# balkce/beamform

Measured on AMD Instinct MI355X. Metric: stft_frames_per_sec, higher is better.
Workload: dtype f64; 1 GPU; das 8-mic 1024-pt (hop 512), 65536-frame batch per GPU, 1 stream(s), planar input resident in HBM; frames_per_gpu=65536, frames_fed_per_gpu=65536, mics=8, fft=1024, hop=512, streams=1, layout=planar, gather=n/a, parallelism=independent batches x1, input=uniform noise in [-0.5, 0.5), settle_launches_before_warmup=408, forward_transforms_per_frame_pair=6

## Files before the change

### beamform_amd/csrc/das_f64_plan.hpp

```cpp
#pragma once

#include <cstdlib>
#include <cstring>

#include "../../include/bfcore.h"

#if defined(__HIPCC__)
#define BF_PLAN_HD __host__ __device__ inline
#else
#define BF_PLAN_HD inline
#endif

namespace bf {

constexpr int kChunkEnd = 0xFFFFF;
constexpr int kMaxChunkPairs = 1000;
constexpr int kSchedMaxChunks = 16384;
constexpr size_t kSchedCounterBytes = 256, kSchedRowBytes = 16;
constexpr size_t das_f64_sched_ws_bytes() { return kSchedCounterBytes + kSchedMaxChunks * kSchedRowBytes; }
constexpr int kDasF64Hop = 512, kDasF64Waves = 8, kDasF64RingSlots = 40;

struct DasSchedPlan {
    int n_levels;
    int cnt[8], size[8];
    int n_chunks;
    int grid;
};

BF_PLAN_HD void das_f64_chunk(const DasSchedPlan &p, long n_frames, int n_streams, int k, int *stream, long *t0, long *n) {
    int lvl = 0, kk = k;
    long pair0 = 0;
    while (lvl < p.n_levels - 1 && kk >= p.cnt[lvl] * n_streams) {
        kk -= p.cnt[lvl] * n_streams;
        pair0 += (long)p.cnt[lvl] * p.size[lvl];
        ++lvl;
    }
    const int s = kk / p.cnt[lvl], j = kk - s * p.cnt[lvl];
    *stream = s;
    *t0 = 2 * (pair0 + (long)j * p.size[lvl]);
    long len = 2L * p.size[lvl];
    if (*t0 + len > n_frames) len = n_frames - *t0;
    *n = len;
}

inline DasSchedPlan das_f64_plan(long n_frames, int n_streams, int n_cus, const char *env) {
    DasSchedPlan p{};
    const long pairs = (n_frames + 1) / 2;
    long nb = (long)n_cus / n_streams;
    if (nb < 1) nb = 1;
    int sizes[8], n_sizes = 0;
    const long share = (pairs + nb - 1) / nb;
    if (env && strchr(env, ',')) {
        const char *c = env;
        while (*c && n_sizes < 8) {
            sizes[n_sizes++] = atoi(c);
            c = strchr(c, ',');
            if (!c) break;
            ++c;
        }
    } else if (!(env && atoi(env) == 0) && share >= 48) {
        long front = (share * 13 / 16) & ~7L;
        long rest = share - front;
        while (front > kMaxChunkPairs && n_sizes < 3) {
            sizes[n_sizes++] = kMaxChunkPairs;
            front -= kMaxChunkPairs;
        }
        if (front > kMaxChunkPairs) { rest += front - kMaxChunkPairs; front = kMaxChunkPairs; }
        sizes[n_sizes++] = (int)front;
        while (n_sizes < 6 && rest >= 24) {
            long sz = (rest / 2) & ~7L;
            if (sz > kMaxChunkPairs) sz = kMaxChunkPairs;
            sizes[n_sizes++] = (int)sz;
            rest -= sz;
        }
        if (rest >= 12) { sizes[n_sizes++] = 4; rest -= 4; }
// ... 77 lines not shown
```

### beamform_amd/csrc/das_f64_w64.hip

```cpp
#include <hip/hip_runtime.h>

#include <type_traits>

#include "launch_trace.hpp"
#include "pipeline_kernels.hpp"
#include "w64_f64_dev.hpp"

namespace bf {

namespace {

constexpr int kBlock = 512;
constexpr int kWaves = kBlock / 64;
constexpr int kHop = 512;
constexpr int kTwD = 2 * (1024 + 4 * kTw2RowW64Rot);
constexpr int oTw = 0;
constexpr int oPlane = kTwD;
constexpr int oGain = oPlane + kWaves * kPlaneD;
constexpr int oCross = oGain + 4 * 2048;
constexpr int oFlag = oCross + 512;
constexpr int kWinRow = 18;
constexpr int oWin = oFlag + 8;
constexpr int kLdsD = oWin + 64 * kWinRow;

typedef volatile __attribute__((address_space(3))) int *lds_flag_t;

template <int LAYOUT>
__global__ __launch_bounds__(kBlock) void das_f64_w64_kernel(DasF64Args a, int frames_per_chunk, int chunks_per_stream) {
    __shared__ __attribute__((aligned(16))) double lds[kLdsD];
    const cx<double> *s_tw1 = reinterpret_cast<const cx<double> *>(lds + oTw);
    const cx<double> *s_tw2 = s_tw1 + 1024;
    const cx<double> *s_gain = reinterpret_cast<const cx<double> *>(lds + oGain);
    float *s_cross = reinterpret_cast<float *>(lds + oCross);
    lds_flag_t s_ready = (lds_flag_t)(lds + oFlag);
    lds_flag_t s_cons = s_ready + kWaves;

    const int tid = threadIdx.x, lane = tid & 63;
    const int w = __builtin_amdgcn_readfirstlane(tid >> 6);
    const int M = a.n_mics, NP = (M + 1) >> 1;
    double *plane = lds + oPlane + w * kPlaneD;
    double *wcol = plane + w64_col_rot(lane);
    double *row16 = plane + (lane & 15) * kRS + 16 * (lane >> 4);

    const int stream = blockIdx.x / chunks_per_stream;
    const long c_in_s = blockIdx.x - (long)stream * chunks_per_stream;
    const double *wrow = lds + oWin + lane * kWinRow;

    const long T0 = c_in_s * frames_per_chunk;
    long T1 = T0 + frames_per_chunk;
    if (T1 > a.n_frames) T1 = a.n_frames;
    const float *xs = a.x + (long)stream * a.stream_stride_x;
    const float *hs = a.hist + (long)stream * M * kHop;
    float *ys = a.y + (long)stream * a.n_frames * kHop;

    float na[16], nb[16];
    auto request = [&](long tt, int p) {
        const int ma = 2 * p, mb = (2 * p + 1 < M) ? 2 * p + 1 : ma;
        if (LAYOUT == 0) {
// ... 6 lines not shown
                na[j] = a1[(unsigned)(64 * j + lane)];
                nb[j] = b1[(unsigned)(64 * j + lane)];
                na[j + 8] = a2[(unsigned)(64 * j + lane)];
                nb[j + 8] = b2[(unsigned)(64 * j + lane)];
            }
        } else {
            const float *s1 = tt >= 1 ? xs + (tt - 1) * (long)kHop * M : hs;
            const float *s2 = xs + tt * (long)kHop * M;
            if ((M & 1) == 0) {
#pragma unroll
                for (int j = 0; j < 8; ++j) {
                    const float2 v1 = *reinterpret_cast<const float2 *>(s1 + (unsigned)((64 * j + lane) * M + ma));
                    const float2 v2 = *reinterpret_cast<const float2 *>(s2 + (unsigned)((64 * j + lane) * M + ma));
                    na[j] = v1.x;
                    nb[j] = v1.y;
                    na[j + 8] = v2.x;
                    nb[j + 8] = v2.y;
                }
            } else {
#pragma unroll
                for (int j = 0; j < 8; ++j) {
                    na[j] = s1[(unsigned)((64 * j + lane) * M + ma)];
                    nb[j] = s1[(unsigned)((64 * j + lane) * M + mb)];
                    na[j + 8] = s2[(unsigned)((64 * j + lane) * M + ma)];
                    nb[j + 8] = s2[(unsigned)((64 * j + lane) * M + mb)];
                }
            }
        }
    };

    const int n_iter = (int)((T1 - T0 + kWaves - 1) / kWaves);
    if (T0 + w < T1) request(T0 + w, 0);
    {
        const f64x2 *tw2 = a.tw, *g2 = a.gains;
        f64x2 *ltw = reinterpret_cast<f64x2 *>(lds + oTw), *lg = reinterpret_cast<f64x2 *>(lds + oGain);
#pragma unroll 4
        for (int i = tid; i < kTwD / 2; i += kBlock) ltw[i] = tw2[i];
#pragma unroll 8
        for (int i = tid; i < NP * 1024; i += kBlock) lg[i] = g2[i];
#pragma unroll 2
        for (int i = tid; i < 1024; i += kBlock) lds[oWin + (i & 63) * kWinRow + (i >> 6)] = a.win[i];
        if (tid < 2 * kWaves) s_ready[tid] = -2;
    }
    __syncthreads();
    for (int it = 0; it < n_iter; ++it) {
        const long t = T0 + (long)it * kWaves + w;
        if (t >= T1) break;

        double Sr[16], Si[16];
        for (int p = 0; p < NP; ++p) {
            double re[16], im[16];
            const bool b_ok = 2 * p + 1 < M;
#pragma unroll
            for (int j = 0; j < 8; ++j) {
                const double w0 = wrow[j], w1 = wrow[j + 8];
                const double t = (double)na[j] * w0, u = (double)na[j + 8];
                re[j] = fma(u, w1, t);
                re[j + 8] = fma(-u, w1, t);
            }
            if (b_ok) {
#pragma unroll
                for (int j = 0; j < 8; ++j) {
                    const double w0 = wrow[j], w1 = wrow[j + 8];
                    const double t = (double)nb[j] * w0, u = (double)nb[j + 8];
                    im[j] = fma(u, w1, t);
                    im[j + 8] = fma(-u, w1, t);
                }
            } else {
#pragma unroll
                for (int j = 0; j < 16; ++j) im[j] = 0.0;
            }
            {
                long tn = t;
                int pn = p + 1;
// ... 119 lines not shown
                float *yn = ys + T1 * kHop;
#pragma unroll
                for (int j = 0; j < 8; ++j) atomicAdd(yn + (unsigned)(64 * j + lane), o[j + 8]);
            } else {
                float *to = a.tail_out + (long)stream * kHop;
#pragma unroll
                for (int j = 0; j < 8; ++j) to[(unsigned)(64 * j + lane)] = o[j + 8];
            }
        }
    }
}


#ifdef BF_PARK_PLAIN
#define BF_PARK_LD(p) (*(const volatile float *)(p))
#else
#define BF_PARK_LD(p) __builtin_nontemporal_load(p)
#endif
constexpr int kGRow = 65;
constexpr int kGMic = 8 * kGRow;
constexpr int kSlots = 64;
constexpr int kTwP = 2 * (960 + 4 * kTw2RowW64Rot);
constexpr int pTw = 0;
constexpr int pPlane = kTwP;
constexpr int pGain = pPlane + kWaves * kPlaneD;
constexpr int pFlag = pGain + 7 * kGMic * 2;
constexpr int kRingR = 32;
constexpr int kRingSlots = kRingR + kWaves;
constexpr int pRing = pFlag + (kSlots + 4) / 2;
constexpr int pWin = pRing + kRingR / 2;
constexpr int kLdsP = pWin + 64 * kWinRow;
static_assert(kLdsP * 8 <= 160 * 1024, "LDS");
static_assert((pGain & 1) == 0 && (pWin & 1) == 0, "16-byte alignment");


typedef volatile __attribute__((address_space(3))) int *lds_int_t;
typedef volatile __attribute__((address_space(3))) unsigned long long *lds_u64_t;
__device__ __forceinline__ int lds_fetch_add(lds_int_t p, int v, int lane) {
    int old = 0;
    if (lane == 0) old = __hip_atomic_fetch_add((__attribute__((address_space(3))) int *)p, v, __ATOMIC_RELAXED, __HIP_MEMORY_SCOPE_WORKGROUP);
    return __builtin_amdgcn_readfirstlane(old);
}
__device__ __forceinline__ unsigned long long lds_fetch_add64(lds_u64_t p, int lane) {
    unsigned long long old = 0;
    if (lane == 0) old = __hip_atomic_fetch_add((__attribute__((address_space(3))) unsigned long long *)p, 1ull, __ATOMIC_RELAXED, __HIP_MEMORY_SCOPE_WORKGROUP);
    const unsigned lo = (unsigned)__builtin_amdgcn_readfirstlane((int)(unsigned)old), hi = (unsigned)__builtin_amdgcn_readfirstlane((int)(unsigned)(old >> 32));
    return ((unsigned long long)hi << 32) | lo;
}
struct DasSched {
    const int4 *chunks;
    unsigned *counter;
    int n_chunks;
};
__device__ __forceinline__ unsigned long long pack_work(unsigned vbase, int chunk, int pairs, int next) {
    return ((unsigned long long)(vbase & 0xFFFFFFu) << 40) | ((unsigned long long)(unsigned)chunk << 20) | ((unsigned long long)(unsigned)pairs << 10) | (unsigned)next;
}
struct PairWork {
    int4 d;
    int pos;
    int len;
    unsigned u;
    bool have;
};
__device__ __forceinline__ int4 load_chunk(const int4 *chunks, int k) {
    const int4 d = chunks[k];
    return int4{__builtin_amdgcn_readfirstlane(d.x), __builtin_amdgcn_readfirstlane(d.y), __builtin_amdgcn_readfirstlane(d.z), k};
}
__device__ __forceinline__ PairWork draw_pair(lds_u64_t work, const DasSched &sc, int lane, const int4 held) {
    PairWork r;
    r.have = false;
    r.d = int4{0, 0, 0, 0};
    r.pos = r.len = 0;
    r.u = 0;
    for (;;) {
        const unsigned long long old = lds_fetch_add64(work, lane);
        const int pos = (int)(old & 1023u), len = (int)((old >> 10) & 1023u), k = (int)((old >> 20) & 0xFFFFFu);
        const unsigned vb = (unsigned)(old >> 40);
        if (k == kChunkEnd) return r;
        if (pos < len) {
            if (k == held.w) r.d = held;
            else r.d = load_chunk(sc.chunks, k);
            r.pos = pos; r.len = len; r.u = vb + (unsigned)pos; r.have = true;
            return r;
        }
        if (pos == len) {
// ... 208 lines not shown
            r.h = ring_slot(jp);
        }
        __builtin_amdgcn_fence(__ATOMIC_ACQUIRE, "workgroup");
        return r;
    };
    auto release_pair = [&](const PairWork &pw, bool has_t) {
        const unsigned u2 = 2u * pw.u;
        (void)lds_fetch_add(s_ring + (u2 & (kRingR - 1)), 2, lane);
        (void)lds_fetch_add(s_ring + ((u2 + 1) & (kRingR - 1)), has_t ? 1 : 2, lane);
        if (pw.pos > 0) (void)lds_fetch_add(s_ring + ((u2 - 1) & (kRingR - 1)), 1, lane);
    };
    auto request_ring_mic = [&](const RingHops &r, int m) { request(r.h + m * kHop, r.a + m * kHop, r.b + m * kHop); };
    auto request_ring_extra = [&](bool on, const RingHops &r) {
        if (!on) {
#pragma unroll
            for (int j = 0; j < 8; ++j) e0[j] = e1[j] = e2[j] = 0.f;
            return;
        }
#pragma unroll
        for (int j = 0; j < 8; ++j) {
            e0[j] = r.h[XM * kHop + (unsigned)(64 * j + lane)];
            e1[j] = r.a[XM * kHop + (unsigned)(64 * j + lane)];
            e2[j] = r.b[XM * kHop + (unsigned)(64 * j + lane)];
        }
    };
    RingHops curR{nullptr, nullptr, nullptr};
    (void)curR;

    BF_STAMP(0);
#ifdef BF_W64_STAMPS
    if (lane == 0 && blockIdx.x < 256) g_stamps[(blockIdx.x * 8 + w) * 64 + 59] = __builtin_amdgcn_s_memtime();
#endif
    PairWork cur;
    cur.d = load_chunk(sc.chunks, (int)blockIdx.x);
    cur.len = (cur.d.z + 1) >> 1;
    const int n_static = cur.len < kWaves ? cur.len : kWaves;
    cur.pos = w;
    cur.u = (unsigned)w;
    cur.have = w < n_static;
    if (LAYOUT == 0 && cur.have) {
        request_pair_mic(cur.d.x, cur.d.y + 2L * w, a.slot_mic[0]);
        request_extra(XM >= 0, cur.d.x, cur.d.y + 2L * w);
    } else {
        request_extra(false, 0, 0);
    }
    {
        const f64x2 *tw2 = a.tw + 64;
        f64x2 *ltw = reinterpret_cast<f64x2 *>(lds + pTw), *lg = reinterpret_cast<f64x2 *>(lds + pGain);
#pragma unroll 4
        for (int i = tid; i < kTwP / 2; i += kBlock) ltw[i] = tw2[i];
        for (int k = 0; k < NT; ++k) {
            const f64x2 *g2 = a.gains_mic + a.slot_mic[k] * kGMic;
#pragma unroll 2
            for (int i = tid; i < kGMic; i += kBlock) lg[k * kGMic + i] = g2[i];
        }
#pragma unroll 2
        for (int i = tid; i < 1024; i += kBlock) lds[pWin + (i & 63) * kWinRow + (i >> 6)] = a.win[i];
        if (tid < kSlots) s_state[tid] = 0;
        if (tid < kRingR) s_ring[tid] = 0;
        if (tid == 0) *s_work = pack_work(0u, (int)blockIdx.x, cur.len, n_static);
    }
    __syncthreads();
    BF_STAMP(1);
    BF_STATS_DECL;
    int it = 0;
    if (!cur.have) {
        cur = draw_pair(s_work, sc, lane, cur.d);
        if (LAYOUT == 0 && cur.have) {
            request_pair_mic(cur.d.x, cur.d.y + 2L * cur.pos, a.slot_mic[0]);
            request_extra(XM >= 0, cur.d.x, cur.d.y + 2L * cur.pos);
        }
    }
    while (cur.have) {
        if constexpr (LAYOUT == 1) {
            curR = prepare_pair(cur);
            request_ring_mic(curR, a.slot_mic[0]);
            request_ring_extra(XM >= 0, curR);
        }
        const int stream = cur.d.x;
        const long T0 = cur.d.y, T1 = T0 + cur.d.z;
        const long tA = T0 + 2L * cur.pos;
        const bool pair = tA + 1 < T1;
        const long tL = pair ? tA + 1 : tA;
        const unsigned u = cur.u;
        const bool has_t = cur.pos + 1 < cur.len, has_h = cur.pos > 0;
        float *ys = a.y + (long)stream * a.n_frames * kHop;
        PairWork nxt;
        nxt.have = false;
        const float *hp0 = a.x + (long)stream * a.stream_stride_x + tA * kHop;
        const float *hist0 = a.hist + (long)stream * M * kHop;
// ... 295 lines not shown
    const float4 *src = reinterpret_cast<const float4 *>(x + s * in_stream_stride + tile * 256 * M);
    const int R = M + 1;
    for (int i = tid; i < 64 * M; i += 256) {
        const float4 v = src[i];
        const int e = 4 * i;
        s_t[(e / M) * R + e % M] = v.x;
        s_t[((e + 1) / M) * R + (e + 1) % M] = v.y;
        s_t[((e + 2) / M) * R + (e + 2) % M] = v.z;
        s_t[((e + 3) / M) * R + (e + 3) % M] = v.w;
    }
    __syncthreads();
    float *dst = out + s * out_stream_stride + tile * 256;
    for (int j = tid; j < 64 * M; j += 256) {
        const int m = j >> 6, q = j & 63;
        const float4 v{s_t[(4 * q) * R + m], s_t[(4 * q + 1) * R + m], s_t[(4 * q + 2) * R + m], s_t[(4 * q + 3) * R + m]};
        reinterpret_cast<float4 *>(dst + (long)m * out_mic_stride)[q] = v;
    }
}

}

static_assert(kWaves == kDasF64Waves && kRingSlots == kDasF64RingSlots && kHop == kDasF64Hop, "das_f64_plan.hpp describes other kernels");
static_assert(sizeof(int4) == kSchedRowBytes, "a row of the chunk table is one int4");

static hipError_t launch_interleaved_to_planar(const float *x, float *out, long n, int n_mics, int n_streams, hipStream_t s) {
    const long tiles = n / 256;
    BF_LAUNCH(interleaved_to_planar_kernel, dim3((unsigned)(tiles * n_streams)), dim3(256), 0, s, x, out, tiles, n_mics, (long)n_mics * n, n, (long)n_mics * n);
    return hipGetLastError();
}

hipError_t enqueue_das_f64(DasF64Args a, const DasF64Launch &d, float *scratch, hipStream_t s, hipEvent_t kev0, hipEvent_t kev1, bool *kev_recorded) {
    hipError_t e = hipSuccess;
    int4 *const chunks = reinterpret_cast<int4 *>(reinterpret_cast<char *>(a.sched_ws) + kSchedCounterBytes);
    const DasSched sc{chunks, reinterpret_cast<unsigned *>(a.sched_ws), d.plan.n_chunks};
    if (d.path == DasF64Path::kMicPair) {
        for (int st = 0; st < a.n_streams && d.runs_per_stream > 1; ++st) {
            e = hipMemset2DAsync(a.y + ((long)st * a.n_frames + d.run_frames) * kHop, (size_t)d.run_frames * kHop * sizeof(float), 0, kHop * sizeof(float), (size_t)d.runs_per_stream - 1, s);
            if (e != hipSuccess) return e;
        }
    } else {
        if (d.path == DasF64Path::kRing) {
            a.ring = scratch; a.ring_bytes = d.scratch_bytes; a.hist_out = nullptr;
        } else if (d.path == DasF64Path::kTranspose) {
            const long n = a.n_frames * kHop;
            float *const hist = scratch + (size_t)a.n_streams * a.n_mics * n;
            if ((e = launch_interleaved_to_planar(a.x, scratch, n, a.n_mics, a.n_streams, s)) != hipSuccess) return e;
            if ((e = launch_interleaved_to_planar(a.hist, hist, kHop, a.n_mics, a.n_streams, s)) != hipSuccess) return e;
            a.x = scratch; a.hist = hist; a.hist_out = nullptr; a.mic_stride = n; a.layout = BF_PLANAR;
        }
        BF_LAUNCH(das_f64_sched_kernel, dim3((unsigned)((sc.n_chunks + kSchedPerBlock - 1) / kSchedPerBlock)), dim3(32 * kSchedPerBlock), 0, s, d.plan, chunks, sc.counter, a.y, a.n_frames, a.n_streams);
        if ((e = hipGetLastError()) != hipSuccess) return e;
    }
    if (kev0 && (e = hipEventRecord(kev0, s)) != hipSuccess) return e;
    if (d.path == DasF64Path::kMicPair)
        BF_LAUNCH(das_f64_w64_kernel<1>, dim3((unsigned)(d.runs_per_stream * a.n_streams)), dim3(kBlock), 0, s, a, (int)d.run_frames, (int)d.runs_per_stream);
    else if (d.path == DasF64Path::kRing)
        BF_LAUNCH(das_f64_ring_kernel, dim3((unsigned)d.plan.grid), dim3(kBlock), 0, s, a, sc);
    else
        BF_LAUNCH(das_f64_pair_kernel, dim3((unsigned)d.plan.grid), dim3(kBlock), 0, s, a, sc);
    if ((e = hipGetLastError()) != hipSuccess) return e;
    if (kev1 && (e = hipEventRecord(kev1, s)) == hipSuccess) *kev_recorded = true;
    return e;
}

}

#ifdef BF_W64_STATS
// ... 10 lines not shown
```

### beamform_amd/csrc/pipeline.hip

```cpp
#include "pipeline.hpp"

#include <hip/hip_runtime.h>

#include <cmath>
#include <vector>

#include "device_mem.hpp"
#include "fft1024.hpp"
#include "pipeline_kernels.hpp"
#include "switches.hpp"

namespace bf {

namespace {

class BinPipelineImpl : public Engine {
    static constexpr int kMaxCols = BF_MAX_INTERF + 1;
   public:
    BinPipelineImpl(const bf_config &c, int n_cus) : cfg_(c), n_cus_(n_cus) {
        M_ = c.n_mics;
        H_ = c.hop;
        N_ = 2 * c.hop;
        NQ_ = problems_per_frame(N_);
        YS_ = yh_stride(N_);
        ks_ = kernel_set(N_);
        MF_ = single_ch_ ? 1 : M_;
        NP_ = (MF_ + 1) / 2;
        S_ = c.n_streams;
        D_ = c.n_dirs > 1 ? c.n_dirs : 1;
        if (time_node_) D_ = M_;
        So_ = S_ * D_;
        R_ = (c.algo == BF_GSS && c.gss_out_sources > 1) ? c.gss_out_sources : 1;
        const bool multi = (c.algo == BF_LCMV || c.algo == BF_GSS);
        KP1_ = multi ? c.n_interf + 1 : 1;
        Phist_ = cov_node_ ? c.past_windows : 0;
        z48_ = cov_node_ && c.precision == BF_PRECISION_MIXED;
        zsz_ = z48_ ? sizeof(z48) : sizeof(f64x2);
    }

// ... 12 lines not shown
        }
        if (cov_node_ && (Phist_ < 1 || Phist_ > 64)) {
            err_ = "past_windows must be in 1..64";
            return BF_EINVAL;
        }
        if (time_node_ && (M_ > 16 || cfg_.gsc_filter_size < 1 || cfg_.gsc_filter_size > 256)) {
            err_ = "gsc is built for up to 16 microphones and filter_size 1..256";
            return M_ > 16 ? BF_ENOSYS : BF_EINVAL;
        }
        if (cfg_.algo == BF_PHASEMPF && (cfg_.smooth_size < 1 || cfg_.smooth_size > 64)) {
            err_ = "smooth_size must be in 1..64";
            return BF_EINVAL;
        }
        ENGINE_HIP(d_tw_.upload(N_ == 1024 ? twiddle_table_32x32<f64x2>() : stockham_twiddles<f64x2>(N_)));
        ENGINE_HIP(d_tw32_.upload(twiddle_table_32x32<f32x2>()));
        ENGINE_HIP(d_win_.upload(sqrt_hann(N_)));
        freqs_ = frequency_vector(N_, cfg_.sample_rate);
        ENGINE_HIP(d_freq_.upload(freqs_));
        skip_lo_ = N_; band_yh_hi_ = NQ_ - 1;
        if (band_node_) {
            int klo = N_, khi = 0;
            for (int q = 1; q < NQ_; ++q) {
                const double f = std::fabs(freqs_[q]);
                if (f >= cfg_.freq_min && f <= cfg_.freq_max) { if (q < klo) klo = q; khi = q; }
            }
            if (khi < N_ / 2 - 2) { skip_lo_ = khi; skip_hi_ = N_ - khi; }
            if (cov_node_ && khi < N_ / 2 - 1 && klo <= khi) { band_yh_lo_ = klo; band_yh_hi_ = khi; }
            else if (cov_node_ && klo > khi) { band_yh_lo_ = 1; band_yh_hi_ = 0; }
        }
        for (auto &b : d_steer_) ENGINE_HIP(b.alloc(steer_elems()));
        if (das_one_launch_shape()) {
            for (auto &t : das_) ENGINE_HIP(t.gains_w64.alloc((size_t)4 * 1024));
            for (auto &t : das_) ENGINE_HIP(t.gains_mic.alloc((size_t)8 * kDasMicGainRows * kDasMicGainRow));
            ENGINE_HIP(d_das_sched_.alloc(das_f64_sched_ws_bytes()));
        }
        if (N_ == 1024) ENGINE_HIP(d_tw_w64_.upload(twiddle_table_w64_rot()));
        for (auto &b : d_hist2_) ENGINE_HIP(b.alloc(hist_elems()));
        for (auto &b : d_tail_) ENGINE_HIP(b.alloc(tail_elems()));
        if (Phist_ > 0) ENGINE_HIP(d_zhist_.alloc(zhist_bytes()));
        if (cfg_.algo == BF_GSS) {
            ENGINE_HIP(d_gssW_.alloc(gss_bytes() / sizeof(f64x2)));
            ENGINE_HIP(hipMemset(d_gssW_.get(), 0, gss_bytes()));
        }
        if (cfg_.algo == BF_PHASEMPF || cfg_.algo == BF_MCRA) ENGINE_HIP(d_mpf_.alloc(mpf_bytes() / sizeof(double)));
        if (cfg_.algo == BF_PHASEMPF) ENGINE_HIP(d_smooth_.alloc(smooth_bytes() / sizeof(double)));
        if (time_node_) ENGINE_HIP(d_nlms_.alloc(nlms_bytes() / sizeof(float)));
        return BF_OK;
    }

    int reset(hipStream_t st) override {
        ENGINE_HIP(hipMemsetAsync(d_hist2_[0].get(), 0, hist_elems() * sizeof(float), st));
        hist_cur_ = 0;
        for (auto &b : d_tail_) ENGINE_HIP(hipMemsetAsync(b.get(), 0, tail_elems() * sizeof(float), st));
        tail_cur_ = 0;
        if (d_zhist_.get()) ENGINE_HIP(hipMemsetAsync(d_zhist_.get(), 0, zhist_bytes(), st));
        if (d_mpf_.get()) ENGINE_HIP(hipMemsetAsync(d_mpf_.get(), 0, mpf_bytes(), st));
        if (d_smooth_.get()) ENGINE_HIP(hipMemsetAsync(d_smooth_.get(), 0, smooth_bytes(), st));
        if (d_nlms_.get()) ENGINE_HIP(hipMemsetAsync(d_nlms_.get(), 0, nlms_bytes(), st));
        gss_reset_mask_ = ~0ull;
        return BF_OK;
    }

    int upload_steering(const std::vector<SteeringSet> &dirs, hipStream_t stream) override {
        const int nc = dirs[0].n_cols, nd = (int)dirs.size();
        if ((size_t)nd * nc * M_ * N_ > steer_elems()) {
            err_ = "steering table larger than the device buffer";
            return BF_EINVAL;
        }
        std::vector<f64x2> t((size_t)nd * N_ * M_ * nc);
        for (int d = 0; d < nd; ++d)
            for (int c = 0; c < nc; ++c)
                for (int m = 0; m < M_; ++m)
                    for (int j = 0; j < N_; ++j) {
                        const cplxd w = dirs[d].at(j, m, c);
                        t[(((size_t)d * nc + c) * M_ + m) * N_ + j] = f64x2{w.real(), w.imag()};
                    }
        const int nxt = steer_cur_ ^ 1;
        std::vector<f64x2> dg64, dgm;
        if (das_one_launch_shape()) {
            dg64 = das_pair_gains_w64_f64(das_pair_gains_t<f64x2>(dirs[0], 4), 4);
            dgm = das_mic_gains_w64_f64(dirs[0], 8);
            das_[nxt].slots = das_f64_slots(dirs[0]);
            ENGINE_HIP(hipMemcpyAsync(das_[nxt].gains_w64.get(), dg64.data(), dg64.size() * sizeof(f64x2), hipMemcpyHostToDevice, stream));
            ENGINE_HIP(hipMemcpyAsync(das_[nxt].gains_mic.get(), dgm.data(), dgm.size() * sizeof(f64x2), hipMemcpyHostToDevice, stream));
        }
        ENGINE_HIP(hipMemcpyAsync(d_steer_[nxt].get(), t.data(), t.size() * sizeof(f64x2), hipMemcpyHostToDevice, stream));
        ENGINE_HIP(hipStreamSynchronize(stream));
        steer_cur_ = nxt;
        steer_dir_stride_ = (long)nc * M_ * N_;
        return BF_OK;
    }

    void on_theta_changed(int dir) override { gss_reset_mask_ |= dir < 0 ? ~0ull : (1ull << dir); }
    void set_columns(int kp1) override {
        KP1_ = kp1;
        gss_reset_mask_ = ~0ull;
    }

    RunSnapshot snapshot_for_run() override {
        RunSnapshot sn;
        sn.kp1 = KP1_;
        sn.gss_reset_mask = gss_reset_mask_;
        sn.steer = d_steer_[steer_cur_].get();
        sn.steer_dir_stride = steer_dir_stride_;
        sn.das = DasSnapshot{das_[steer_cur_].gains_w64.get(), das_[steer_cur_].gains_mic.get(), das_[steer_cur_].slots};
        gss_reset_mask_ = 0;
        return sn;
    }
    int columns() const override { return KP1_; }
    unsigned long long pending_resets() const override { return gss_reset_mask_; }
    void set_pending_resets(unsigned long long mask) override { gss_reset_mask_ = mask; }

    int run(const float *x, long F, float *y, f64x2 *spectrum, hipStream_t stream, int layout, long mic_stride,
            const RunSnapshot &snap) override;

    size_t state_bytes() const override {
        return (hist_elems() + tail_elems()) * sizeof(float) + zhist_bytes() + gss_bytes() + mpf_bytes() + smooth_bytes() +
               nlms_bytes();
    }
    int get_state(void *host) override { return copy_state((char *)host, true); }
    int set_state(const void *host) override { return copy_state((char *)host, false); }

   private:
    static constexpr int kDeclined = 1;
    int run_das_one_launch(const float *x, long F, float *y, hipStream_t stream, int layout, long mic_stride, const RunSnapshot &snap);
    int run_chain(const float *x, long F, float *y, f64x2 *spectrum, hipStream_t stream, int layout, long mic_stride, const RunSnapshot &snap);
    bool das_one_launch_shape() const { return cfg_.algo == BF_DAS && N_ == 1024 && M_ <= 8 && D_ == 1; }
    size_t steer_elems() const { return (size_t)D_ * N_ * M_ * kMaxCols; }
    size_t hist_elems() const { return (size_t)S_ * M_ * H_; }
    size_t tail_elems() const { return (size_t)So_ * R_ * H_; }
    size_t zhist_bytes() const { return Phist_ ? (size_t)S_ * Phist_ * NP_ * N_ * zsz_ : 0; }
    size_t gss_bytes() const { return cfg_.algo == BF_GSS ? (size_t)So_ * N_ * kMaxCols * M_ * sizeof(f64x2) : 0; }
    size_t mpf_bytes() const {
        return (cfg_.algo == BF_PHASEMPF || cfg_.algo == BF_MCRA) ? (size_t)So_ * (kMpfVecs * N_ + 8) * sizeof(double) : 0;
    }
    size_t smooth_bytes() const { return cfg_.algo == BF_PHASEMPF ? (size_t)So_ * 64 * sizeof(double) : 0; }
    size_t nlms_bytes() const {
        return time_node_ ? (size_t)S_ * (2 * (M_ - 1) + 1) * cfg_.gsc_filter_size * sizeof(float) : 0;
// ... 6 lines not shown
            {d_zhist_.get(), zhist_bytes()}, {d_gssW_.get(), gss_bytes()}, {d_mpf_.get(), mpf_bytes()}, {d_smooth_.get(), smooth_bytes()},
            {d_nlms_.get(), nlms_bytes()}};
        for (auto &s : segs) {
            if (!s.n) continue;
            if (to_host)
                ENGINE_HIP(hipMemcpy(p, s.d, s.n, hipMemcpyDeviceToHost));
            else
                ENGINE_HIP(hipMemcpy(s.d, p, s.n, hipMemcpyHostToDevice));
            p += s.n;
        }
        return BF_OK;
    }

    bf_config cfg_;
    int n_cus_, M_, MF_, NP_, S_, D_, So_, R_, KP1_, Phist_;
    const bool cov_node_ = cfg_.algo == BF_MVDR || cfg_.algo == BF_LCMV;
    const bool band_node_ = cov_node_ || cfg_.algo == BF_GSS;
    const bool time_node_ = cfg_.algo == BF_GSC;
    const bool single_ch_ = cfg_.algo == BF_MCRA;
    const bool post_amp_ = band_node_;
    const bool yraw_target_ = cfg_.algo == BF_PHASEMPF || time_node_;
    int skip_lo_, skip_hi_ = 0;
    int band_yh_lo_ = 0, band_yh_hi_;
    bool z48_ = false;
    size_t zsz_ = sizeof(f64x2);
    int H_ = 512, N_ = 1024, NQ_ = 514, YS_ = 516;
    const KernelSet *ks_ = nullptr;
    long steer_dir_stride_ = 0;
    std::vector<double> freqs_;
    DeviceBuffer<f64x2> d_tw_;
    DeviceBuffer<f32x2> d_tw32_;
    DeviceBuffer<double> d_win_, d_freq_;
    DeviceBuffer<f64x2> d_steer_[2];
    struct DasTables { DeviceBuffer<f64x2> gains_w64, gains_mic; DasSlots slots; } das_[2];
    DeviceBuffer<f64x2> d_tw_w64_;
    DeviceBuffer<char> d_das_sched_;
    int steer_cur_ = 0;
    DeviceBuffer<float> d_hist2_[2];
    int hist_cur_ = 0;
    DeviceBuffer<float> d_tail_[2];
    int tail_cur_ = 0;
    DeviceBuffer<char> d_zhist_;
    DeviceBuffer<f64x2> d_gssW_;
    DeviceBuffer<double> d_mpf_;
    DeviceBuffer<double> d_smooth_;
    DeviceBuffer<float> d_nlms_;
    unsigned long long gss_reset_mask_ = ~0ull;
    DeviceBuffer<char> d_Z_;
    DeviceBuffer<char> d_Yh_;
    DeviceBuffer<float> d_yraw_;
    DeviceBuffer<float> d_planar_;
    DeviceBuffer<float> d_frames_;
};

int BinPipelineImpl::run_das_one_launch(const float *x, long F, float *y, hipStream_t stream, int layout, long mic_stride, const RunSnapshot &snap) {
    const Switches &sw = switches();
    if (!das_one_launch_shape() || sw.fused_bins != 1 || snap.das.gains_w64 == nullptr) return kDeclined;
    const DasSlots &sl = snap.das.slots;
    const DasF64Launch d = das_f64_decide(DasF64Shape{layout, M_, S_, n_cus_, F, sl.mic0_unit, snap.das.gains_mic && d_das_sched_.get(), sl.n_tr,
                                                      sw.das_il_ring, sw.das_f64_sched});
    if (d.path == DasF64Path::kChain) return kDeclined;
    ENGINE_HIP(d_planar_.reserve((d.scratch_bytes + sizeof(float) - 1) / sizeof(float)));
    float *const hist = d_hist2_[hist_cur_].get();
    DasF64Args da;
    da.x = x; da.hist = hist; da.hist_out = d_hist2_[hist_cur_ ^ 1].get(); da.y = y;
    da.tail_in = d_tail_[tail_cur_].get(); da.tail_out = d_tail_[tail_cur_ ^ 1].get();
    da.win = d_win_.get(); da.n_frames = F; da.mic_stride = mic_stride;
    da.stream_stride_x = (long)M_ * F * H_; da.n_streams = S_; da.n_mics = M_; da.run_len = 1; da.layout = layout;
    da.gains = snap.das.gains_w64; da.gains_mic = snap.das.gains_mic; da.tw = d_tw_w64_.get();
    da.mic0_unit = sl.mic0_unit ? 1 : 0; da.n_tr = sl.n_tr; da.extra_mic = sl.extra_mic;
    for (int k = 0; k < 8; ++k) da.slot_mic[k] = sl.slot_mic[k];
    da.sched_ws = d_das_sched_.get(); da.sched_ws_bytes = d_das_sched_.get() ? das_f64_sched_ws_bytes() : 0;
    ENGINE_HIP(enqueue_das_f64(da, d, d_planar_.get(), stream, kev0, kev1, &kev_recorded));
    if (d.writes_hist)
        hist_cur_ ^= 1;
    else
        ENGINE_HIP(carry_last_hop(hist, x, F, H_, M_, S_, layout, mic_stride, (long)F * H_ * M_, stream));
    tail_cur_ ^= 1;
    return BF_OK;
}

int BinPipelineImpl::run(const float *x, long F, float *y, f64x2 *spectrum, hipStream_t stream, int layout, long mic_stride,
                         const RunSnapshot &snap) {
    const int rc = spectrum ? kDeclined : run_das_one_launch(x, F, y, stream, layout, mic_stride, snap);
    return rc == kDeclined ? run_chain(x, F, y, spectrum, stream, layout, mic_stride, snap) : rc;
}

int BinPipelineImpl::run_chain(const float *x, long F, float *y, f64x2 *spectrum, hipStream_t stream, int layout, long mic_stride,
                               const RunSnapshot &snap) {
    const Switches &sw = switches();
    const ChainPlan p = chain_decide(ChainShape{cfg_.algo, N_, layout, M_, S_, cfg_.n_dirs > 1 ? cfg_.n_dirs : 1, snap.kp1, cfg_.past_windows,
                                                cfg_.precision, spectrum != nullptr, F, n_cus_, cfg_.gsc_filter_size, cfg_.smooth_size,
                                                band_yh_lo_, band_yh_hi_, (reinterpret_cast<size_t>(y) & 15) == 0, sw.fused_bins,
                                                sw.stft_small, sw.stft_split, sw.mvdr_group, sw.gss_group, sw.gsc_serial, R_});
    float *const hist = d_hist2_[hist_cur_].get();
    const long FT = Phist_ + F;
    ENGINE_HIP(d_Z_.reserve(p.z_bytes));
    ENGINE_HIP(d_Yh_.reserve(p.yh_bytes));
    ENGINE_HIP(d_yraw_.reserve(p.yraw_elems));
    ENGINE_HIP(d_frames_.reserve(p.frames_elems));
    f64x2 *const Z = (f64x2 *)d_Z_.get();
    f64x2 *const Yh = (f64x2 *)d_Yh_.get();
// ... 73 lines not shown
```

### beamform_amd/csrc/pipeline.hpp

```cpp
#pragma once

#include <hip/hip_runtime.h>

#include <string>
#include <vector>

#include "../../include/bfcore.h"
#include "geometry.hpp"

namespace bf {

struct DasSnapshot {
    const f64x2 *gains_w64 = nullptr, *gains_mic = nullptr;
    DasSlots slots;
};

struct RunSnapshot {
    int kp1 = 1;
    unsigned long long gss_reset_mask = 0;
    const f64x2 *steer = nullptr;
    long steer_dir_stride = 0;
    DasSnapshot das;
};

class Engine {
   public:
    static Engine *create(const bf_config &cfg, int n_cus);
    virtual ~Engine() {}
    virtual int init() = 0;
    virtual int reset(hipStream_t stream) = 0;
    virtual int upload_steering(const std::vector<SteeringSet> &dirs, hipStream_t stream) = 0;
    virtual void on_theta_changed(int dir = -1) = 0;
    virtual void set_columns(int kp1) = 0;
    virtual RunSnapshot snapshot_for_run() = 0;
    virtual int run(const float *x_dev, long n_frames, float *y_dev, f64x2 *spectrum_dev, hipStream_t stream, int layout,
                    long mic_stride, const RunSnapshot &snap) = 0;
    virtual int columns() const = 0;
    virtual unsigned long long pending_resets() const = 0;
    virtual void set_pending_resets(unsigned long long mask) = 0;
    virtual size_t state_bytes() const = 0;
    virtual int get_state(void *host) = 0;
    virtual int set_state(const void *host) = 0;
    const std::string &error() const { return err_; }
    hipEvent_t kev0 = nullptr, kev1 = nullptr;
    bool kev_recorded = false;

   protected:
// ... 16 lines not shown
```

### beamform_amd/csrc/pipeline_kernels.hpp

```cpp
#pragma once

#include <hip/hip_runtime.h>

#include "../../include/bfcore.h"
#include "chain_plan.hpp"
#include "das_f64_plan.hpp"
#include "geometry.hpp"

namespace bf {

#ifdef BF_NFFT
#define BF_CAT2_(a, b) a##b
#define BF_CAT2(a, b) BF_CAT2_(a, b)
#define BF_NTAG BF_CAT2(n, BF_NFFT)
#endif

constexpr int problems_per_frame(int nfft) { return nfft / 2 + 2; }
constexpr int yh_stride(int nfft) { return nfft / 2 + 4; }
constexpr int kMpfVecs = 7;
#ifdef BF_NFFT
namespace BF_NTAG {
constexpr int kN = BF_NFFT;
constexpr int kHop = kN / 2;
constexpr int kNQ = problems_per_frame(kN);
// ... 49 lines not shown
    int gss_rows = 1;
};
struct IstftArgs {
    const f64x2 *Yh;
    int yh32;
    int yh_lo, yh_hi;
    float *y;
    const float *tail_in;
    float *tail_out;
    const f64x2 *tw;
    const f32x2 *tw32;
    const f64x2 *tw_w64 = nullptr;
    float *frames;
    const double *win;
    long n_frames;
    int n_streams;
    double post_amp;
    int use_post_amp;
};
struct DasF64Args {
    const float *x;
    const float *hist;
    float *y;
    const float *tail_in;
    float *tail_out;
    const f64x2 *gains;
    const f64x2 *tw;
    const double *win;
    long n_frames, mic_stride, stream_stride_x;
    int n_streams, n_mics, run_len;
    int layout = 0;
    float *hist_out = nullptr;
    const f64x2 *gains_mic = nullptr;
    int n_tr = 0, extra_mic = -1;
    int slot_mic[8] = {1, 2, 3, 4, 5, 6, 7, 0};
    int mic0_unit = 0;
    void *sched_ws = nullptr;
    size_t sched_ws_bytes = 0;
    float *ring = nullptr;
    size_t ring_bytes = 0;
};

hipError_t enqueue_das_f64(DasF64Args a, const DasF64Launch &d, float *scratch, hipStream_t s, hipEvent_t kev0, hipEvent_t kev1, bool *kev_recorded);

#ifdef BF_NFFT
namespace BF_NTAG {
hipError_t launch_stft(const ChainPlan &p, const StftArgs &a, int n_cus, hipStream_t s);
hipError_t launch_bins(const ChainPlan &p, const BinsArgs &a, int n_cus, hipStream_t s);
hipError_t launch_stft_bins_fused(const ChainPlan &p, const StftArgs &a, const BinsArgs &b, int n_cus, hipStream_t s);
hipError_t launch_pointwise(const ChainPlan &p, const BinsArgs &a, hipStream_t s);
hipError_t launch_mpf_mask(const ChainPlan &p, const BinsArgs &a, hipStream_t s);
hipError_t launch_mcra_node(const BinsArgs &a, hipStream_t s);
hipError_t launch_mvdr_lcmv(const ChainPlan &p, const BinsArgs &a, int n_cus, hipStream_t s);
hipError_t launch_gss(const ChainPlan &p, const BinsArgs &a, hipStream_t s);
hipError_t launch_gsc_align(const BinsArgs &a, hipStream_t s);
hipError_t launch_bins_end(const ChainPlan &p, const BinsArgs &a, hipStream_t s);
hipError_t launch_expand_spectrum(const f64x2 *Yh, f64x2 *spectrum, long frames, hipStream_t s);
hipError_t launch_istft(const ChainPlan &p, const IstftArgs &a, int n_cus, hipStream_t s);
hipError_t launch_gsc_nlms(const ChainPlan &p, const float *aligned, float *y, float *state, long n_samples, int n_streams, int n_mics,
                           const bf_config &cfg, hipStream_t s);
hipError_t launch_smooth(const ChainPlan &p, const float *yraw, float *y, double *state, long n_frames, int n_streams, hipStream_t s);
}
#endif

struct KernelSet {
    int nfft;
// ... 29 lines not shown
```

Before: 135.5 million frames/s.

## Preload DAS LDS tables from precomputed host images with batched register staging

Builds host-side packed images of the twiddles, the pre-transposed window and the per-slot mic gains, so the frame-pair kernel's prologue copies contiguous arrays into LDS. All global loads are issued into registers before any LDS store, instead of interleaving load/store loops. The first chunk is computed arithmetically from the schedule plan instead of being read from the chunk table. This shortens the per-block startup latency, at the cost of an extra device buffer, a host upload on each steering change, and more registers in the prologue.

```diff
diff --git a/beamform_amd/csrc/das_f64_image.hpp b/beamform_amd/csrc/das_f64_image.hpp
--- /dev/null
+++ b/beamform_amd/csrc/das_f64_image.hpp
@@ -0,0 +1,42 @@
+#pragma once
+
+#include <vector>
+
+#include "das_f64_plan.hpp"
+#include "geometry.hpp"
+
+namespace bf {
+
+constexpr int kDasImgThreads = 512;
+constexpr int kDasImgWinRow = 18;
+constexpr int kDasImgTw = 960 + 4 * kTw2RowW64Rot;
+constexpr int kDasImgWin = 64 * kDasImgWinRow / 2;
+constexpr int kDasImgStatic = kDasImgTw + kDasImgWin;
+constexpr int kDasImgGainMic = kDasMicGainRows * kDasMicGainRow;
+constexpr int kDasImgMaxSlots = 7;
+constexpr int kDasImgGains = kDasImgMaxSlots * kDasImgGainMic;
+constexpr int das_f64_image_slots(int len) { return (len + kDasImgThreads - 1) / kDasImgThreads; }
+constexpr int kDasImgTwSlots = das_f64_image_slots(kDasImgTw);
+constexpr int kDasImgWinSlots = das_f64_image_slots(kDasImgWin);
+constexpr int kDasImgGainSlots = das_f64_image_slots(kDasImgGains);
+
+BF_PLAN_HD int das_f64_image_elem(int s, int tid) { return s * kDasImgThreads + tid; }
+BF_PLAN_HD int das_f64_image_src(int elem, int len) { return elem < len ? elem : len - 1; }
+
+inline std::vector<f64x2> das_f64_image_static(const std::vector<f64x2> &tw_w64_rot, const std::vector<double> &win) {
+    std::vector<f64x2> img(kDasImgStatic, f64x2{0.0, 0.0});
+    for (int i = 0; i < kDasImgTw; ++i) img[i] = tw_w64_rot[64 + i];
+    std::vector<double> rows((size_t)64 * kDasImgWinRow, 0.0);
+    for (int i = 0; i < 1024; ++i) rows[(size_t)(i & 63) * kDasImgWinRow + (i >> 6)] = win[i];
+    for (int i = 0; i < kDasImgWin; ++i) img[kDasImgTw + i] = f64x2{rows[2 * i], rows[2 * i + 1]};
+    return img;
+}
+
+inline std::vector<f64x2> das_f64_image_gains(const std::vector<f64x2> &gains_mic, const DasSlots &sl) {
+    std::vector<f64x2> img(kDasImgGains, f64x2{0.0, 0.0});
+    for (int k = 0; k < sl.n_tr && k < kDasImgMaxSlots; ++k)
+        for (int i = 0; i < kDasImgGainMic; ++i) img[(size_t)k * kDasImgGainMic + i] = gains_mic[(size_t)sl.slot_mic[k] * kDasImgGainMic + i];
+    return img;
+}
+
+}
diff --git a/beamform_amd/csrc/das_f64_plan.hpp b/beamform_amd/csrc/das_f64_plan.hpp
--- a/beamform_amd/csrc/das_f64_plan.hpp
+++ b/beamform_amd/csrc/das_f64_plan.hpp
@@ -41,6 +41,14 @@
     long len = 2L * p.size[lvl];
     if (*t0 + len > n_frames) len = n_frames - *t0;
     *n = len;
+}
+
+struct DasChunkRow { int stream, t0, n; };
+BF_PLAN_HD DasChunkRow das_f64_first_chunk(const DasSchedPlan &p, long n_frames, int n_streams, int b) {
+    int stream;
+    long t0, n;
+    das_f64_chunk(p, n_frames, n_streams, b, &stream, &t0, &n);
+    return DasChunkRow{stream, (int)t0, (int)n};
 }
 
 inline DasSchedPlan das_f64_plan(long n_frames, int n_streams, int n_cus, const char *env) {
diff --git a/beamform_amd/csrc/das_f64_w64.hip b/beamform_amd/csrc/das_f64_w64.hip
--- a/beamform_amd/csrc/das_f64_w64.hip
+++ b/beamform_amd/csrc/das_f64_w64.hip
@@ -2,6 +2,7 @@
 
 #include <type_traits>
 
+#include "das_f64_image.hpp"
 #include "launch_trace.hpp"
 #include "pipeline_kernels.hpp"
 #include "w64_f64_dev.hpp"
@@ -24,6 +25,8 @@
 constexpr int kLdsD = oWin + 64 * kWinRow;
 
 typedef volatile __attribute__((address_space(3))) int *lds_flag_t;
+typedef double tab2 __attribute__((ext_vector_type(2)));
+static_assert(kBlock == kDasImgThreads, "das_f64_image.hpp's copy schedule is one of 512 threads");
 
 template <int LAYOUT>
 __global__ __launch_bounds__(kBlock) void das_f64_w64_kernel(DasF64Args a, int frames_per_chunk, int chunks_per_stream) {
@@ -96,14 +99,36 @@
     const int n_iter = (int)((T1 - T0 + kWaves - 1) / kWaves);
     if (T0 + w < T1) request(T0 + w, 0);
     {
-        const f64x2 *tw2 = a.tw, *g2 = a.gains;
-        f64x2 *ltw = reinterpret_cast<f64x2 *>(lds + oTw), *lg = reinterpret_cast<f64x2 *>(lds + oGain);
-#pragma unroll 4
-        for (int i = tid; i < kTwD / 2; i += kBlock) ltw[i] = tw2[i];
-#pragma unroll 8
-        for (int i = tid; i < NP * 1024; i += kBlock) lg[i] = g2[i];
-#pragma unroll 2
-        for (int i = tid; i < 1024; i += kBlock) lds[oWin + (i & 63) * kWinRow + (i >> 6)] = a.win[i];
+        constexpr int kTwN = kTwD / 2, kTwS = (kTwN + kBlock - 1) / kBlock, kGS = 4 * 1024 / kBlock;
+        const tab2 *tw2 = reinterpret_cast<const tab2 *>(a.tw), *g2 = reinterpret_cast<const tab2 *>(a.gains);
+        tab2 *ltw = reinterpret_cast<tab2 *>(lds + oTw), *lg = reinterpret_cast<tab2 *>(lds + oGain);
+        const int n_g = NP * 1024;
+        tab2 v_tw[kTwS], v_g[kGS];
+        double v_w[1024 / kBlock];
+        int ct = tid;
+        asm volatile("" : "+v"(ct));
+#pragma unroll
+        for (int s = 0; s < kTwS; ++s) v_tw[s] = tw2[das_f64_image_src(das_f64_image_elem(s, ct), kTwN)];
+#pragma unroll
+        for (int s = 0; s < kGS; ++s) v_g[s] = g2[das_f64_image_src(das_f64_image_elem(s, ct), n_g)];
+#pragma unroll
+        for (int s = 0; s < 1024 / kBlock; ++s) v_w[s] = a.win[das_f64_image_elem(s, ct)];
+        BF_STAGE();
+#pragma unroll
+        for (int s = 0; s < kTwS; ++s) {
+            const int i = das_f64_image_elem(s, ct);
+            if (i < kTwN) ltw[i] = v_tw[s];
+        }
+#pragma unroll
+        for (int s = 0; s < kGS; ++s) {
+            const int i = das_f64_image_elem(s, ct);
+            if (i < n_g) lg[i] = v_g[s];
+        }
+#pragma unroll
+        for (int s = 0; s < 1024 / kBlock; ++s) {
+            const int i = das_f64_image_elem(s, ct);
+            lds[oWin + (i & 63) * kWinRow + (i >> 6)] = v_w[s];
+        }
         if (tid < 2 * kWaves) s_ready[tid] = -2;
     }
     __syncthreads();
@@ -289,6 +314,7 @@
 constexpr int kLdsP = pWin + 64 * kWinRow;
 static_assert(kLdsP * 8 <= 160 * 1024, "LDS");
 static_assert((pGain & 1) == 0 && (pWin & 1) == 0, "16-byte alignment");
+static_assert(kTwP == 2 * kDasImgTw && kGMic == kDasImgGainMic && kWinRow == kDasImgWinRow && pFlag == pGain + 2 * kDasImgGains, "das_f64_image.hpp describes another LDS map");
 
 
 typedef volatile __attribute__((address_space(3))) int *lds_int_t;
@@ -308,6 +334,7 @@
     const int4 *chunks;
     unsigned *counter;
     int n_chunks;
+    DasSchedPlan plan;
 };
 __device__ __forceinline__ unsigned long long pack_work(unsigned vbase, int chunk, int pairs, int next) {
     return ((unsigned long long)(vbase & 0xFFFFFFu) << 40) | ((unsigned long long)(unsigned)chunk << 20) | ((unsigned long long)(unsigned)pairs << 10) | (unsigned)next;
@@ -582,7 +609,10 @@
     if (lane == 0 && blockIdx.x < 256) g_stamps[(blockIdx.x * 8 + w) * 64 + 59] = __builtin_amdgcn_s_memtime();
 #endif
     PairWork cur;
-    cur.d = load_chunk(sc.chunks, (int)blockIdx.x);
+    {
+        const DasChunkRow r0 = das_f64_first_chunk(sc.plan, a.n_frames, a.n_streams, (int)blockIdx.x);
+        cur.d = int4{r0.stream, r0.t0, r0.n, (int)blockIdx.x};
+    }
     cur.len = (cur.d.z + 1) >> 1;
     const int n_static = cur.len < kWaves ? cur.len : kWaves;
     cur.pos = w;
@@ -595,17 +625,32 @@
         request_extra(false, 0, 0);
     }
     {
-        const f64x2 *tw2 = a.tw + 64;
-        f64x2 *ltw = reinterpret_cast<f64x2 *>(lds + pTw), *lg = reinterpret_cast<f64x2 *>(lds + pGain);
-#pragma unroll 4
-        for (int i = tid; i < kTwP / 2; i += kBlock) ltw[i] = tw2[i];
-        for (int k = 0; k < NT; ++k) {
-            const f64x2 *g2 = a.gains_mic + a.slot_mic[k] * kGMic;
-#pragma unroll 2
-            for (int i = tid; i < kGMic; i += kBlock) lg[k * kGMic + i] = g2[i];
-        }
-#pragma unroll 2
-        for (int i = tid; i < 1024; i += kBlock) lds[pWin + (i & 63) * kWinRow + (i >> 6)] = a.win[i];
+        const tab2 *i_tw = reinterpret_cast<const tab2 *>(a.img_static), *i_win = i_tw + kDasImgTw, *i_g = reinterpret_cast<const tab2 *>(a.img_gains);
+        tab2 *ltw = reinterpret_cast<tab2 *>(lds + pTw), *lwin = reinterpret_cast<tab2 *>(lds + pWin), *lg = reinterpret_cast<tab2 *>(lds + pGain);
+        const int n_g = NT * kDasImgGainMic;
+        tab2 v_tw[kDasImgTwSlots], v_win[kDasImgWinSlots], v_g[kDasImgGainSlots];
+#pragma unroll
+        for (int s = 0; s < kDasImgTwSlots; ++s) v_tw[s] = i_tw[das_f64_image_src(das_f64_image_elem(s, tid), kDasImgTw)];
+#pragma unroll
+        for (int s = 0; s < kDasImgWinSlots; ++s) v_win[s] = i_win[das_f64_image_src(das_f64_image_elem(s, tid), kDasImgWin)];
+#pragma unroll
+        for (int s = 0; s < kDasImgGainSlots; ++s) v_g[s] = i_g[das_f64_image_src(das_f64_image_elem(s, tid), n_g)];
+        BF_STAGE();
+#pragma unroll
+        for (int s = 0; s < kDasImgTwSlots; ++s) {
+            const int i = das_f64_image_elem(s, tid);
+            if (i < kDasImgTw) ltw[i] = v_tw[s];
+        }
+#pragma unroll
+        for (int s = 0; s < kDasImgWinSlots; ++s) {
+            const int i = das_f64_image_elem(s, tid);
+            if (i < kDasImgWin) lwin[i] = v_win[s];
+        }
+#pragma unroll
+        for (int s = 0; s < kDasImgGainSlots; ++s) {
+            const int i = das_f64_image_elem(s, tid);
+            if (i < n_g) lg[i] = v_g[s];
+        }
         if (tid < kSlots) s_state[tid] = 0;
         if (tid < kRingR) s_ring[tid] = 0;
         if (tid == 0) *s_work = pack_work(0u, (int)blockIdx.x, cur.len, n_static);
@@ -967,7 +1012,7 @@
 hipError_t enqueue_das_f64(DasF64Args a, const DasF64Launch &d, float *scratch, hipStream_t s, hipEvent_t kev0, hipEvent_t kev1, bool *kev_recorded) {
     hipError_t e = hipSuccess;
     int4 *const chunks = reinterpret_cast<int4 *>(reinterpret_cast<char *>(a.sched_ws) + kSchedCounterBytes);
-    const DasSched sc{chunks, reinterpret_cast<unsigned *>(a.sched_ws), d.plan.n_chunks};
+    const DasSched sc{chunks, reinterpret_cast<unsigned *>(a.sched_ws), d.plan.n_chunks, d.plan};
     if (d.path == DasF64Path::kMicPair) {
         for (int st = 0; st < a.n_streams && d.runs_per_stream > 1; ++st) {
             e = hipMemset2DAsync(a.y + ((long)st * a.n_frames + d.run_frames) * kHop, (size_t)d.run_frames * kHop * sizeof(float), 0, kHop * sizeof(float), (size_t)d.runs_per_stream - 1, s);
diff --git a/beamform_amd/csrc/pipeline.hip b/beamform_amd/csrc/pipeline.hip
--- a/beamform_amd/csrc/pipeline.hip
+++ b/beamform_amd/csrc/pipeline.hip
@@ -5,6 +5,7 @@
 #include <cmath>
 #include <vector>
 
+#include "das_f64_image.hpp"
 #include "device_mem.hpp"
 #include "fft1024.hpp"
 #include "pipeline_kernels.hpp"
@@ -83,7 +84,9 @@
         if (das_one_launch_shape()) {
             for (auto &t : das_) ENGINE_HIP(t.gains_w64.alloc((size_t)4 * 1024));
             for (auto &t : das_) ENGINE_HIP(t.gains_mic.alloc((size_t)8 * kDasMicGainRows * kDasMicGainRow));
+            for (auto &t : das_) ENGINE_HIP(t.img_gains.alloc((size_t)kDasImgGains));
             ENGINE_HIP(d_das_sched_.alloc(das_f64_sched_ws_bytes()));
+            ENGINE_HIP(d_das_img_.upload(das_f64_image_static(twiddle_table_w64_rot(), sqrt_hann(N_))));
         }
         if (N_ == 1024) ENGINE_HIP(d_tw_w64_.upload(twiddle_table_w64_rot()));
         for (auto &b : d_hist2_) ENGINE_HIP(b.alloc(hist_elems()));
@@ -127,11 +130,13 @@
                         t[(((size_t)d * nc + c) * M_ + m) * N_ + j] = f64x2{w.real(), w.imag()};
                     }
         const int nxt = steer_cur_ ^ 1;
-        std::vector<f64x2> dg64, dgm;
+        std::vector<f64x2> dg64, dgm, dimg;
         if (das_one_launch_shape()) {
             dg64 = das_pair_gains_w64_f64(das_pair_gains_t<f64x2>(dirs[0], 4), 4);
             dgm = das_mic_gains_w64_f64(dirs[0], 8);
             das_[nxt].slots = das_f64_slots(dirs[0]);
+            dimg = das_f64_image_gains(dgm, das_[nxt].slots);
+            ENGINE_HIP(hipMemcpyAsync(das_[nxt].img_gains.get(), dimg.data(), dimg.size() * sizeof(f64x2), hipMemcpyHostToDevice, stream));
             ENGINE_HIP(hipMemcpyAsync(das_[nxt].gains_w64.get(), dg64.data(), dg64.size() * sizeof(f64x2), hipMemcpyHostToDevice, stream));
             ENGINE_HIP(hipMemcpyAsync(das_[nxt].gains_mic.get(), dgm.data(), dgm.size() * sizeof(f64x2), hipMemcpyHostToDevice, stream));
         }
@@ -154,7 +159,7 @@
         sn.gss_reset_mask = gss_reset_mask_;
         sn.steer = d_steer_[steer_cur_].get();
         sn.steer_dir_stride = steer_dir_stride_;
-        sn.das = DasSnapshot{das_[steer_cur_].gains_w64.get(), das_[steer_cur_].gains_mic.get(), das_[steer_cur_].slots};
+        sn.das = DasSnapshot{das_[steer_cur_].gains_w64.get(), das_[steer_cur_].gains_mic.get(), das_[steer_cur_].slots, das_[steer_cur_].img_gains.get()};
         gss_reset_mask_ = 0;
         return sn;
     }
@@ -227,7 +232,8 @@
     DeviceBuffer<f32x2> d_tw32_;
     DeviceBuffer<double> d_win_, d_freq_;
     DeviceBuffer<f64x2> d_steer_[2];
-    struct DasTables { DeviceBuffer<f64x2> gains_w64, gains_mic; DasSlots slots; } das_[2];
+    struct DasTables { DeviceBuffer<f64x2> gains_w64, gains_mic, img_gains; DasSlots slots; } das_[2];
+    DeviceBuffer<f64x2> d_das_img_;
     DeviceBuffer<f64x2> d_tw_w64_;
     DeviceBuffer<char> d_das_sched_;
     int steer_cur_ = 0;
@@ -252,7 +258,7 @@
     const Switches &sw = switches();
     if (!das_one_launch_shape() || sw.fused_bins != 1 || snap.das.gains_w64 == nullptr) return kDeclined;
     const DasSlots &sl = snap.das.slots;
-    const DasF64Launch d = das_f64_decide(DasF64Shape{layout, M_, S_, n_cus_, F, sl.mic0_unit, snap.das.gains_mic && d_das_sched_.get(), sl.n_tr,
+    const DasF64Launch d = das_f64_decide(DasF64Shape{layout, M_, S_, n_cus_, F, sl.mic0_unit, snap.das.gains_mic && snap.das.img_gains && d_das_img_.get() && d_das_sched_.get(), sl.n_tr,
                                                       sw.das_il_ring, sw.das_f64_sched});
     if (d.path == DasF64Path::kChain) return kDeclined;
     ENGINE_HIP(d_planar_.reserve((d.scratch_bytes + sizeof(float) - 1) / sizeof(float)));
@@ -263,6 +269,7 @@
     da.win = d_win_.get(); da.n_frames = F; da.mic_stride = mic_stride;
     da.stream_stride_x = (long)M_ * F * H_; da.n_streams = S_; da.n_mics = M_; da.run_len = 1; da.layout = layout;
     da.gains = snap.das.gains_w64; da.gains_mic = snap.das.gains_mic; da.tw = d_tw_w64_.get();
+    da.img_static = d_das_img_.get(); da.img_gains = snap.das.img_gains;
     da.mic0_unit = sl.mic0_unit ? 1 : 0; da.n_tr = sl.n_tr; da.extra_mic = sl.extra_mic;
     for (int k = 0; k < 8; ++k) da.slot_mic[k] = sl.slot_mic[k];
     da.sched_ws = d_das_sched_.get(); da.sched_ws_bytes = d_das_sched_.get() ? das_f64_sched_ws_bytes() : 0;
diff --git a/beamform_amd/csrc/pipeline.hpp b/beamform_amd/csrc/pipeline.hpp
--- a/beamform_amd/csrc/pipeline.hpp
+++ b/beamform_amd/csrc/pipeline.hpp
@@ -13,6 +13,7 @@
 struct DasSnapshot {
     const f64x2 *gains_w64 = nullptr, *gains_mic = nullptr;
     DasSlots slots;
+    const f64x2 *img_gains = nullptr;
 };
 
 struct RunSnapshot {
diff --git a/beamform_amd/csrc/pipeline_kernels.hpp b/beamform_amd/csrc/pipeline_kernels.hpp
--- a/beamform_amd/csrc/pipeline_kernels.hpp
+++ b/beamform_amd/csrc/pipeline_kernels.hpp
@@ -105,6 +105,7 @@
     int layout = 0;
     float *hist_out = nullptr;
     const f64x2 *gains_mic = nullptr;
+    const f64x2 *img_static = nullptr, *img_gains = nullptr;
     int n_tr = 0, extra_mic = -1;
     int slot_mic[8] = {1, 2, 3, 4, 5, 6, 7, 0};
     int mic0_unit = 0;
```

Measured after the change: 136.8 million frames/s (median of 6 runs). About the same (+0.9%).
